# CFSAN-Biostatistics/snp-pipeline

Measured on AMD Instinct MI355X. Metric: consensus_bases_called_per_sec, higher is better.
Workload: dtype u8; 1 GPU; BASELINE configs[3] shard (125 samples/GPU x 5000000 bp x 30x synthetic pileups, 49878 SNP sites, 1500 SNP records per sample; the reference bundles no pileups); step = site-record gather + site union, one batched scan launch + one call launch, 4-bit pack, row all-gather, all-pairs distance tiles, row-band exchange; samples_total=125, samples_this_rank=125, genome_bp=5000000, snp_sites=49878, pileup_bytes_this_rank=54061520755, parallelism=samples sharded over 1 rank(s)

## Files before the change

snp_pipeline_amd/csrc/prims.h:

```cpp
#pragma once

#include <hip/hip_runtime.h>
#include <stdint.h>

__device__ __forceinline__ uint32_t wave_inclusive_sum(uint32_t v) {
    v += (uint32_t)__builtin_amdgcn_update_dpp(0, (int)v, 0x111, 0xF, 0xF, false);
    v += (uint32_t)__builtin_amdgcn_update_dpp(0, (int)v, 0x112, 0xF, 0xF, false);
    v += (uint32_t)__builtin_amdgcn_update_dpp(0, (int)v, 0x114, 0xF, 0xF, false);
    v += (uint32_t)__builtin_amdgcn_update_dpp(0, (int)v, 0x118, 0xF, 0xF, false);
    v += (uint32_t)__builtin_amdgcn_update_dpp(0, (int)v, 0x142, 0xA, 0xF, false);
    v += (uint32_t)__builtin_amdgcn_update_dpp(0, (int)v, 0x143, 0xC, 0xF, false);
    return v;
}

__device__ __forceinline__ uint32_t block_exclusive_sum(uint32_t v, uint32_t *lds, uint32_t &total) {
    const uint32_t lane = threadIdx.x & 63, wave = threadIdx.x >> 6, n_waves = (blockDim.x + 63) >> 6;
    const uint32_t incl = wave_inclusive_sum(v);
    if (lane == 63) lds[wave] = incl;
    __syncthreads();
    if (wave == 0) {
        const uint32_t w = lane < n_waves ? lds[lane] : 0u;
        const uint32_t wi = wave_inclusive_sum(w);
        if (lane < n_waves) lds[lane] = wi - w;
        if (lane == 63) lds[16] = wi;
    }
    __syncthreads();
    total = lds[16];
    return lds[wave] + incl - v;
}

#define PRIM_SCAN_THREADS 1024
#define PRIM_SCAN_ITEMS 8
#define PRIM_SCAN_BLOCK (PRIM_SCAN_THREADS * PRIM_SCAN_ITEMS)

static inline uint32_t prim_scan_blocks(uint64_t n) { return (uint32_t)((n + PRIM_SCAN_BLOCK - 1) / PRIM_SCAN_BLOCK); }
static inline size_t prim_scan_workspace_words(uint64_t n) { return (size_t)prim_scan_blocks(n) + 2; }

__global__ __launch_bounds__(PRIM_SCAN_THREADS) static void k_prim_scan_reduce(const uint32_t *in, uint64_t n, uint32_t *block_sums) {
    __shared__ uint32_t lds[17];
    const uint64_t base = (uint64_t)blockIdx.x * PRIM_SCAN_BLOCK + (uint64_t)threadIdx.x * PRIM_SCAN_ITEMS;
    uint32_t s = 0;
#pragma unroll
    for (int k = 0; k < PRIM_SCAN_ITEMS; ++k) s += base + k < n ? in[base + k] : 0u;
    uint32_t total;
    (void)block_exclusive_sum(s, lds, total);
    if (threadIdx.x == 0) block_sums[blockIdx.x] = total;
}

__global__ __launch_bounds__(PRIM_SCAN_THREADS) static void k_prim_scan_spine(uint32_t *block_sums, uint32_t n_blocks, uint32_t *total) {
    __shared__ uint32_t lds[17];
    uint32_t carry = 0;
    for (uint32_t b0 = 0; b0 < n_blocks; b0 += PRIM_SCAN_THREADS) {
        const uint32_t i = b0 + threadIdx.x;
        const uint32_t v = i < n_blocks ? block_sums[i] : 0u;
        uint32_t t;
        const uint32_t ex = block_exclusive_sum(v, lds, t);
        if (i < n_blocks) block_sums[i] = carry + ex;
        carry += t;
        __syncthreads();
    }
    if (threadIdx.x == 0) total[0] = carry;
}

__global__ __launch_bounds__(PRIM_SCAN_THREADS) static void k_prim_scan_apply(const uint32_t *in, uint32_t *out, uint64_t n, const uint32_t *block_sums) {
    __shared__ uint32_t lds[17];
    const uint64_t base = (uint64_t)blockIdx.x * PRIM_SCAN_BLOCK + (uint64_t)threadIdx.x * PRIM_SCAN_ITEMS;
    uint32_t v[PRIM_SCAN_ITEMS], s = 0;
#pragma unroll
    for (int k = 0; k < PRIM_SCAN_ITEMS; ++k) { v[k] = base + k < n ? in[base + k] : 0u; s += v[k]; }
    uint32_t total;
    uint32_t run = block_sums[blockIdx.x] + block_exclusive_sum(s, lds, total);
#pragma unroll
    for (int k = 0; k < PRIM_SCAN_ITEMS; ++k) {
        if (base + k < n) out[base + k] = run;
        run += v[k];
    }
}

static inline void prim_exclusive_scan_u32(hipStream_t st, const uint32_t *in, uint32_t *out, uint64_t n, uint32_t *ws, uint32_t **d_total) {
    const uint32_t nb = prim_scan_blocks(n);
    uint32_t *total = ws + nb;
    if (d_total) *d_total = total;
    if (n == 0) { (void)hipMemsetAsync(total, 0, 4, st); return; }
    k_prim_scan_reduce<<<nb, PRIM_SCAN_THREADS, 0, st>>>(in, n, ws);
    k_prim_scan_spine<<<1, PRIM_SCAN_THREADS, 0, st>>>(ws, nb, total);
    k_prim_scan_apply<<<nb, PRIM_SCAN_THREADS, 0, st>>>(in, out, n, ws);
}

#define PRIM_GSCAN_THREADS 256
#define PRIM_GSCAN_ITEMS 8
#define PRIM_GSCAN_BLOCK (PRIM_GSCAN_THREADS * PRIM_GSCAN_ITEMS)
static inline uint32_t prim_gscan_blocks(uint64_t n) { return (uint32_t)((n + PRIM_GSCAN_BLOCK - 1) / PRIM_GSCAN_BLOCK); }

template <typename T, typename Op>
__device__ __forceinline__ T block_inclusive_scan_generic(T v, T *lds, Op op) {
    lds[threadIdx.x] = v;
    __syncthreads();
    for (uint32_t d = 1; d < PRIM_GSCAN_THREADS; d <<= 1) {
        T other = v;
        const bool take = threadIdx.x >= d;
        if (take) other = lds[threadIdx.x - d];
        __syncthreads();
        if (take) { v = op(other, v); lds[threadIdx.x] = v; }
        __syncthreads();
    }
    return v;
}

template <typename T, typename Op, int kPhase>
__global__ __launch_bounds__(PRIM_GSCAN_THREADS) static void k_prim_gscan(const T *in, T *out, uint64_t n, T *aggr, uint32_t n_blocks, Op op) {
    __shared__ T lds[PRIM_GSCAN_THREADS];
    if (kPhase == 1) {
        T carry = T();
        bool have = false;
        for (uint32_t b0 = 0; b0 < n_blocks; b0 += PRIM_GSCAN_THREADS) {
            const uint32_t i = b0 + threadIdx.x;
            const uint32_t last = n_blocks - b0 < PRIM_GSCAN_THREADS ? n_blocks - b0 - 1 : PRIM_GSCAN_THREADS - 1;
            T v = aggr[i < n_blocks ? i : n_blocks - 1];
            if (i >= n_blocks) v = aggr[n_blocks - 1];
            T s = block_inclusive_scan_generic(v, lds, op);
            if (have) s = op(carry, s);
            if (i < n_blocks) aggr[i] = s;
            __syncthreads();
            lds[threadIdx.x] = s;
            __syncthreads();
            carry = lds[last];
            have = true;
            __syncthreads();
        }
        return;
    }
    const uint64_t base = (uint64_t)blockIdx.x * PRIM_GSCAN_BLOCK + (uint64_t)threadIdx.x * PRIM_GSCAN_ITEMS;
    T v[PRIM_GSCAN_ITEMS];
    const uint64_t left = base < n ? n - base : 0;
    const int cnt = left >= PRIM_GSCAN_ITEMS ? PRIM_GSCAN_ITEMS : (int)left;
#pragma unroll
    for (int k = 0; k < PRIM_GSCAN_ITEMS; ++k) if (k < cnt) v[k] = in[base + k];
#pragma unroll
    for (int k = 1; k < PRIM_GSCAN_ITEMS; ++k) if (k < cnt) v[k] = op(v[k - 1], v[k]);
    __shared__ uint8_t ok[PRIM_GSCAN_THREADS];
    ok[threadIdx.x] = cnt > 0;
    T a = cnt > 0 ? v[cnt - 1] : T();
    lds[threadIdx.x] = a;
    __syncthreads();
    bool a_ok = cnt > 0;
    for (uint32_t d = 1; d < PRIM_GSCAN_THREADS; d <<= 1) {
        T other = a;
        bool o_ok = false;
        const bool take = threadIdx.x >= d;
        if (take) { other = lds[threadIdx.x - d]; o_ok = ok[threadIdx.x - d]; }
        __syncthreads();
        if (take && o_ok) { a = a_ok ? op(other, a) : other; a_ok = true; lds[threadIdx.x] = a; ok[threadIdx.x] = 1; }
        __syncthreads();
    }
    if (kPhase == 0) {
        if (threadIdx.x == PRIM_GSCAN_THREADS - 1) aggr[blockIdx.x] = a;
        return;
    }
    T pre = T();
    bool pre_ok = false;
    if (threadIdx.x > 0) { pre = lds[threadIdx.x - 1]; pre_ok = ok[threadIdx.x - 1]; }
    if (blockIdx.x > 0) { const T bp = aggr[blockIdx.x - 1]; pre = pre_ok ? op(bp, pre) : bp; pre_ok = true; }
#pragma unroll
    for (int k = 0; k < PRIM_GSCAN_ITEMS; ++k) if (k < cnt) out[base + k] = pre_ok ? op(pre, v[k]) : v[k];
}

template <typename T, typename Op>
static inline void prim_inclusive_scan(hipStream_t st, const T *in, T *out, uint64_t n, T *aggr, Op op) {
    if (n == 0) return;
    const uint32_t nb = prim_gscan_blocks(n);
    k_prim_gscan<T, Op, 0><<<nb, PRIM_GSCAN_THREADS, 0, st>>>(in, out, n, aggr, nb, op);
    k_prim_gscan<T, Op, 1><<<1, PRIM_GSCAN_THREADS, 0, st>>>(in, out, n, aggr, nb, op);
    k_prim_gscan<T, Op, 2><<<nb, PRIM_GSCAN_THREADS, 0, st>>>(in, out, n, aggr, nb, op);
}

#define PRIM_SORT_TILE 2048
#ifndef PRIM_SORT_THREADS
#define PRIM_SORT_THREADS 1024
#endif

template <typename T, typename Less>
__global__ __launch_bounds__(PRIM_SORT_THREADS) static void k_prim_sort_check(const T *in, uint64_t n, uint32_t *unsorted, Less less) {
    bool bad = false;
    for (uint64_t i = (uint64_t)blockIdx.x * blockDim.x + threadIdx.x; i + 1 < n; i += (uint64_t)gridDim.x * blockDim.x)
        bad = bad || less(in[i + 1], in[i]);
    if (__ballot(bad) && (threadIdx.x & 63) == 0) *unsorted = 1u;
}

template <typename T, typename Less>
__global__ __launch_bounds__(PRIM_SORT_THREADS) static void k_prim_sort_tiles(const T *in, T *out, T *out_if_sorted, uint64_t n,
                                                                             const uint32_t *unsorted, Less less) {
    __shared__ T tile[PRIM_SORT_TILE];
    __shared__ uint16_t idx[PRIM_SORT_TILE];
    const uint64_t base = (uint64_t)blockIdx.x * PRIM_SORT_TILE;
    const uint32_t cnt = n - base < PRIM_SORT_TILE ? (uint32_t)(n - base) : PRIM_SORT_TILE;
    if (*unsorted == 0) {
        for (uint32_t i = threadIdx.x; i < cnt; i += PRIM_SORT_THREADS) out_if_sorted[base + i] = in[base + i];
        return;
    }
    for (uint32_t i = threadIdx.x; i < PRIM_SORT_TILE; i += PRIM_SORT_THREADS) {
        if (i < cnt) tile[i] = in[base + i];
        idx[i] = i < cnt ? (uint16_t)i : (uint16_t)0xFFFFu;
    }
    __syncthreads();
    auto before = [&](uint16_t a, uint16_t b) -> bool {
        if (a == 0xFFFFu || b == 0xFFFFu) return a != 0xFFFFu && b == 0xFFFFu;
        if (less(tile[a], tile[b])) return true;
        if (less(tile[b], tile[a])) return false;
        return a < b;
    };
    for (uint32_t k = 2; k <= PRIM_SORT_TILE; k <<= 1)
        for (uint32_t j = k >> 1; j > 0; j >>= 1) {
            for (uint32_t t = threadIdx.x; t < PRIM_SORT_TILE / 2; t += PRIM_SORT_THREADS) {
                const uint32_t lo = ((t & ~(j - 1)) << 1) | (t & (j - 1)), hi = lo | j;
                const bool up = (lo & k) == 0;
                const uint16_t a = idx[lo], b = idx[hi];
                if (before(b, a) == up) { idx[lo] = b; idx[hi] = a; }
            }
            __syncthreads();
        }
    for (uint32_t i = threadIdx.x; i < cnt; i += PRIM_SORT_THREADS) out[base + i] = tile[idx[i]];
}

template <typename T, typename Less>
__global__ __launch_bounds__(PRIM_SORT_THREADS) static void k_prim_merge_pass(const T *in, T *out, uint64_t n, uint64_t run,
                                                                             const uint32_t *unsorted, Less less) {
    __shared__ T stage[PRIM_SORT_TILE];
    __shared__ uint64_t split[2];
    if (*unsorted == 0) return;
    const uint64_t o0 = (uint64_t)blockIdx.x * PRIM_SORT_TILE;
    const uint64_t pair0 = o0 / (2 * run) * (2 * run);
    const uint64_t a_begin = pair0, a_len = n - pair0 < run ? n - pair0 : run;
    const uint64_t b_begin = pair0 + a_len, b_len = n - b_begin < run ? n - b_begin : run;
    const uint64_t d0 = o0 - pair0, total = a_len + b_len;
    const uint64_t d1 = d0 + PRIM_SORT_TILE < total ? d0 + PRIM_SORT_TILE : total;
    const T *A = in + a_begin, *B = in + b_begin;
    if (threadIdx.x < 2) {
        const uint64_t d = threadIdx.x ? d1 : d0;
        uint64_t lo = d > b_len ? d - b_len : 0, hi = d < a_len ? d : a_len;
        while (lo < hi) {
            const uint64_t mid = (lo + hi) >> 1;
            if (!less(B[d - 1 - mid], A[mid])) lo = mid + 1; else hi = mid;
        }
        split[threadIdx.x] = lo;
    }
    __syncthreads();
    const uint64_t a0 = split[0], a1 = split[1], b0 = d0 - a0, b1 = d1 - a1;
    const uint32_t na = (uint32_t)(a1 - a0), nb = (uint32_t)(b1 - b0);
    for (uint32_t i = threadIdx.x; i < na + nb; i += PRIM_SORT_THREADS) stage[i] = i < na ? A[a0 + i] : B[b0 + (i - na)];
    __syncthreads();
    for (uint32_t i = threadIdx.x; i < na + nb; i += PRIM_SORT_THREADS) {
        const T v = stage[i];
        uint32_t lo, hi;
        if (i < na) {
            lo = 0; hi = nb;
            while (lo < hi) { const uint32_t mid = (lo + hi) >> 1; if (less(stage[na + mid], v)) lo = mid + 1; else hi = mid; }
            out[o0 + i + lo] = v;
        } else {
            lo = 0; hi = na;
            while (lo < hi) { const uint32_t mid = (lo + hi) >> 1; if (!less(v, stage[mid])) lo = mid + 1; else hi = mid; }
            out[o0 + (i - na) + lo] = v;
        }
    }
}

static inline uint32_t prim_sort_passes(uint64_t n) {
    uint32_t p = 0;
    for (uint64_t run = PRIM_SORT_TILE; run < n; run <<= 1) ++p;
    return p;
}
template <typename T, typename Less>
static inline T *prim_sort(hipStream_t st, const T *in, T *buf_a, T *buf_b, uint64_t n, uint32_t *flag, Less less) {
    const uint32_t passes = prim_sort_passes(n);
    T *final_buf = (passes & 1) ? buf_b : buf_a;
    if (n == 0) return final_buf;
    const uint32_t tiles = (uint32_t)((n + PRIM_SORT_TILE - 1) / PRIM_SORT_TILE);
    (void)hipMemsetAsync(flag, 0, 4, st);
    const uint64_t cb = (n + PRIM_SORT_THREADS - 1) / PRIM_SORT_THREADS;
    k_prim_sort_check<T, Less><<<(unsigned)(cb < 2048 ? cb : 2048), PRIM_SORT_THREADS, 0, st>>>(in, n, flag, less);
    k_prim_sort_tiles<T, Less><<<tiles, PRIM_SORT_THREADS, 0, st>>>(in, buf_a, final_buf, n, flag, less);
    T *src = buf_a, *dst = buf_b;
    for (uint64_t run = PRIM_SORT_TILE; run < n; run <<= 1) {
        k_prim_merge_pass<T, Less><<<tiles, PRIM_SORT_THREADS, 0, st>>>(src, dst, n, run, flag, less);
        T *t = src; src = dst; dst = t;
    }
    return final_buf;
}
```

snp_pipeline_amd/csrc/regions.hip:

```cpp
#include <string.h>

#include <vector>

#include "internal.h"
#include "prims.h"

namespace {

inline size_t up256(size_t x) { return (x + 255) / 256 * 256; }
inline unsigned nblk(uint64_t n) { return (unsigned)((n + 255) / 256); }

#define R_TRY(ctx, expr)                                                                                \
    do {                                                                                                \
        hipError_t e_ = (expr);                                                                         \
        if (e_ != hipSuccess)                                                                           \
            return snpgpu_set_error((ctx), SNPGPU_E_HIP, "%s failed: %s", #expr, hipGetErrorString(e_)); \
    } while (0)

#define REG_ERR_POSITION 1u
#define REG_ERR_INTERVAL 2u

struct U64Less { __device__ bool operator()(const uint64_t &a, const uint64_t &b) const { return a < b; } };

#define MAX_RULES 64
struct Rules { int32_t max_snps[MAX_RULES], window[MAX_RULES]; uint32_t n; };

__device__ __forceinline__ uint32_t seg_of(const uint32_t *seg_off, uint32_t n_segs, uint32_t i) {
    uint32_t lo = 0, hi = n_segs;
    while (hi - lo > 1) { uint32_t mid = (lo + hi) >> 1; if (seg_off[mid] <= i) lo = mid; else hi = mid; }
    return lo;
}

__global__ void k_seg_keys(const int64_t *pos, const uint32_t *seg_off, uint32_t n_segs, uint32_t n_pos, uint64_t *keys, uint32_t *out_n) {
    uint32_t i = blockIdx.x * blockDim.x + threadIdx.x;
    if (i >= n_pos) return;
    int64_t p = pos[i];
    if (p < 0 || p >= (1ll << 40)) { atomicOr(&out_n[1], REG_ERR_POSITION); p = 0; }
    keys[i] = ((uint64_t)seg_of(seg_off, n_segs, i) << 40) | (uint64_t)p;
}

__global__ void k_dense_flags(const uint64_t *keys, const uint32_t *seg_off, uint32_t n_segs, uint32_t n_pos, Rules rules, uint32_t *flag) {
    uint64_t g = (uint64_t)blockIdx.x * blockDim.x + threadIdx.x;
    if (g >= (uint64_t)n_pos * rules.n) return;
    const uint32_t i = (uint32_t)(g / rules.n), r = (uint32_t)(g % rules.n);
    const uint32_t end = seg_off[seg_of(seg_off, n_segs, i) + 1];
    const int64_t m = rules.max_snps[r], mask = (1ll << 40) - 1;
    uint32_t f = 0;
    if (m >= 0 && (uint64_t)i + (uint64_t)m < end) f = ((int64_t)(keys[i] & mask) + (int64_t)rules.window[r] - 1 >= (int64_t)(keys[i + m] & mask)) ? 1u : 0u;
    flag[g] = f;
}

__global__ void k_dense_emit(const uint64_t *keys, uint32_t n_pos, Rules rules, const uint32_t *flag, const uint32_t *slot,
                             int64_t *out_start, int64_t *out_end, uint32_t *out_seg) {
    uint64_t g = (uint64_t)blockIdx.x * blockDim.x + threadIdx.x;
    if (g >= (uint64_t)n_pos * rules.n || !flag[g]) return;
    const uint32_t i = (uint32_t)(g / rules.n), r = (uint32_t)(g % rules.n);
    const uint64_t mask = (1ull << 40) - 1;
    const uint32_t o = slot[g];
    out_start[o] = (int64_t)(keys[i] & mask);
    out_end[o] = (int64_t)(keys[i + rules.max_snps[r]] & mask);
    out_seg[o] = (uint32_t)(keys[i] >> 40);
}

__global__ void k_copy_word(const uint32_t *src, uint32_t *dst) { *dst = *src; }

size_t dense_ws_bytes(uint32_t n_pos, uint32_t n_rules) {
    const uint64_t total = (uint64_t)n_pos * n_rules;
    return 3 * up256(8ull * n_pos) + 256 + 2 * up256(4 * total) + up256(4 * prim_scan_workspace_words(total)) + 256;
}

int dense_enqueue(snpgpu_ctx *ctx, const int64_t *d_pos, const uint32_t *d_seg_off, uint32_t n_segs, uint32_t n_pos, const Rules &rules,
                  int64_t *d_out_start, int64_t *d_out_end, uint32_t *d_out_seg, uint32_t *d_out_n, char *ws) {
    hipStream_t st = ctx->stream;
    const uint64_t total = (uint64_t)n_pos * rules.n;
    size_t o = 0;
    uint64_t *keys = (uint64_t *)(ws + o); o += up256(8ull * n_pos);
    uint64_t *ka = (uint64_t *)(ws + o); o += up256(8ull * n_pos);
    uint64_t *kb = (uint64_t *)(ws + o); o += up256(8ull * n_pos);
    uint32_t *sflag = (uint32_t *)(ws + o); o += 256;
    uint32_t *flag = (uint32_t *)(ws + o); o += up256(4 * total);
    uint32_t *slot = (uint32_t *)(ws + o); o += up256(4 * total);
    uint32_t *scan_ws = (uint32_t *)(ws + o);
    R_TRY(ctx, hipMemsetAsync(d_out_n, 0, 8, st));
    if (n_pos && rules.n) {
        k_seg_keys<<<nblk(n_pos), 256, 0, st>>>(d_pos, d_seg_off, n_segs, n_pos, keys, d_out_n);
        const uint64_t *sorted = prim_sort<uint64_t, U64Less>(st, keys, ka, kb, n_pos, sflag, U64Less());
        k_dense_flags<<<nblk(total), 256, 0, st>>>(sorted, d_seg_off, n_segs, n_pos, rules, flag);
        uint32_t *d_total = nullptr;
        prim_exclusive_scan_u32(st, flag, slot, total, scan_ws, &d_total);
        k_dense_emit<<<nblk(total), 256, 0, st>>>(sorted, n_pos, rules, flag, slot, d_out_start, d_out_end, d_out_seg);
        k_copy_word<<<1, 1, 0, st>>>(d_total, d_out_n);
    }
    R_TRY(ctx, hipGetLastError());
    return SNPGPU_OK;
}

int make_rules(snpgpu_ctx *ctx, const int32_t *max_snps, const int32_t *window, uint32_t n_rules, Rules &rules) {
    if (n_rules > MAX_RULES) return snpgpu_set_error(ctx, SNPGPU_E_UNSUPPORTED, "more than %d dense-window rules", MAX_RULES);
    if (n_rules && (!max_snps || !window)) return snpgpu_set_error(ctx, SNPGPU_E_ARG, "null dense-window argument");
    memset(&rules, 0, sizeof rules);
    rules.n = n_rules;
    for (uint32_t r = 0; r < n_rules; ++r) { rules.max_snps[r] = max_snps[r]; rules.window[r] = window[r]; }
    return SNPGPU_OK;
}

struct Ival { uint32_t group, pad; int64_t start, end; };
struct IvalLess {
    __device__ bool operator()(const Ival &a, const Ival &b) const {
        if (a.group != b.group) return a.group < b.group;
        if (a.start != b.start) return a.start < b.start;
        return a.end < b.end;
    }
};
struct GroupMax { int64_t maxend; uint32_t group, pad; };
struct GroupMaxOp {
    __device__ GroupMax operator()(const GroupMax &a, const GroupMax &b) const {
        GroupMax r;
        r.group = b.group; r.pad = 0;
        r.maxend = (a.group == b.group && a.maxend > b.maxend) ? a.maxend : b.maxend;
        return r;
    }
};

__global__ void k_ival_pack(const uint32_t *group, const int64_t *start, const int64_t *end, uint32_t n, Ival *out, uint32_t *out_n) {
    uint32_t i = blockIdx.x * blockDim.x + threadIdx.x;
    if (i >= n) return;
    Ival v;
    v.group = group[i]; v.pad = 0; v.start = start[i]; v.end = end[i];
    if (v.start > v.end) atomicOr(&out_n[1], REG_ERR_INTERVAL);
    out[i] = v;
}

__global__ void k_ival_ends(const Ival *sorted, uint32_t n, GroupMax *gm) {
    uint32_t i = blockIdx.x * blockDim.x + threadIdx.x;
    if (i < n) { GroupMax g; g.group = sorted[i].group; g.pad = 0; g.maxend = sorted[i].end; gm[i] = g; }
}

__global__ void k_ival_heads(const Ival *sorted, const GroupMax *run, uint32_t n, uint32_t *head) {
    uint32_t i = blockIdx.x * blockDim.x + threadIdx.x;
    if (i >= n) return;
    uint32_t h = 1;
    if (i > 0 && run[i - 1].group == sorted[i].group) {
        const int64_t le = run[i - 1].maxend;
        h = (le == INT64_MAX || sorted[i].start <= le + 1) ? 0u : 1u;
    }
    head[i] = h;
}

__global__ void k_ival_emit(const Ival *sorted, const GroupMax *run, const uint32_t *head, const uint32_t *slot, uint32_t n,
                            uint32_t *out_group, int64_t *out_start, int64_t *out_end) {
    uint32_t i = blockIdx.x * blockDim.x + threadIdx.x;
    if (i >= n) return;
    const uint32_t o = slot[i] + head[i] - 1;
    if (head[i]) { out_group[o] = sorted[i].group; out_start[o] = sorted[i].start; }
    if (i + 1 == n || head[i + 1]) out_end[o] = run[i].maxend;
}

size_t merge_regions_ws_bytes(uint32_t n) {
    return 3 * up256(sizeof(Ival) * (size_t)n) + 256 + 2 * up256(sizeof(GroupMax) * (size_t)n) + up256(sizeof(GroupMax) * (size_t)prim_gscan_blocks(n)) +
           2 * up256(4ull * n) + up256(4 * prim_scan_workspace_words(n)) + 256;
}

int merge_regions_enqueue(snpgpu_ctx *ctx, const uint32_t *d_group, const int64_t *d_start, const int64_t *d_end, uint32_t n,
                          uint32_t *d_out_group, int64_t *d_out_start, int64_t *d_out_end, uint32_t *d_out_n, char *ws) {
    hipStream_t st = ctx->stream;
    size_t o = 0;
    Ival *iv = (Ival *)(ws + o); o += up256(sizeof(Ival) * (size_t)n);
    Ival *ia = (Ival *)(ws + o); o += up256(sizeof(Ival) * (size_t)n);
    Ival *ib = (Ival *)(ws + o); o += up256(sizeof(Ival) * (size_t)n);
    uint32_t *sflag = (uint32_t *)(ws + o); o += 256;
    GroupMax *gm = (GroupMax *)(ws + o); o += up256(sizeof(GroupMax) * (size_t)n);
    GroupMax *run = (GroupMax *)(ws + o); o += up256(sizeof(GroupMax) * (size_t)n);
    GroupMax *aggr = (GroupMax *)(ws + o); o += up256(sizeof(GroupMax) * (size_t)prim_gscan_blocks(n));
    uint32_t *head = (uint32_t *)(ws + o); o += up256(4ull * n);
    uint32_t *slot = (uint32_t *)(ws + o); o += up256(4ull * n);
    uint32_t *scan_ws = (uint32_t *)(ws + o);
    R_TRY(ctx, hipMemsetAsync(d_out_n, 0, 8, st));
    if (n) {
        k_ival_pack<<<nblk(n), 256, 0, st>>>(d_group, d_start, d_end, n, iv, d_out_n);
        const Ival *sorted = prim_sort<Ival, IvalLess>(st, iv, ia, ib, n, sflag, IvalLess());
        k_ival_ends<<<nblk(n), 256, 0, st>>>(sorted, n, gm);
        prim_inclusive_scan<GroupMax, GroupMaxOp>(st, gm, run, n, aggr, GroupMaxOp());
        k_ival_heads<<<nblk(n), 256, 0, st>>>(sorted, run, n, head);
        uint32_t *d_total = nullptr;
        prim_exclusive_scan_u32(st, head, slot, n, scan_ws, &d_total);
        k_ival_emit<<<nblk(n), 256, 0, st>>>(sorted, run, head, slot, n, d_out_group, d_out_start, d_out_end);
        k_copy_word<<<1, 1, 0, st>>>(d_total, d_out_n);
    }
    R_TRY(ctx, hipGetLastError());
    return SNPGPU_OK;
}

__global__ void k_in_regions(const uint32_t *pos_group, const int64_t *pos, uint32_t n, const uint32_t *reg_off,
                             const int64_t *rs, const int64_t *re, uint32_t n_groups, uint8_t *out) {
    uint32_t i = blockIdx.x * blockDim.x + threadIdx.x;
    if (i >= n) return;
    uint32_t g = pos_group[i];
    uint8_t f = 0;
    if (g < n_groups) {
        int64_t p = pos[i];
        uint32_t lo = reg_off[g], hi = reg_off[g + 1];
        while (lo < hi) {
            uint32_t mid = (lo + hi) >> 1;
            if (rs[mid] <= p) lo = mid + 1; else hi = mid;
        }
        if (lo > reg_off[g]) f = re[lo - 1] >= p;
    }
    out[i] = f;
}

struct Pair { uint64_t key; uint32_t samp, pad; };
struct PairLess {
    __device__ bool operator()(const Pair &a, const Pair &b) const { return a.key != b.key ? a.key < b.key : a.samp < b.samp; }
};

__global__ void k_pair_pack(const uint64_t *keys, const uint32_t *samp, uint32_t n, Pair *out) {
    uint32_t i = blockIdx.x * blockDim.x + threadIdx.x;
    if (i < n) { Pair p; p.key = keys[i]; p.samp = samp[i]; p.pad = 0; out[i] = p; }
}

__global__ void k_sites_flags(const Pair *sorted, uint32_t n, uint32_t *new_key, uint32_t *new_pair) {
    uint32_t i = blockIdx.x * blockDim.x + threadIdx.x;
    if (i >= n) return;
    const bool nk = i == 0 || sorted[i].key != sorted[i - 1].key;
    new_key[i] = nk;
    new_pair[i] = nk || sorted[i].samp != sorted[i - 1].samp;
}

__global__ void k_sites_emit(const Pair *sorted, uint32_t n, const uint32_t *new_key, const uint32_t *new_pair, const uint32_t *key_slot,
                             const uint32_t *pair_slot, const uint32_t *n_keys, const uint32_t *n_pairs, uint64_t *out_unique,
                             uint32_t *out_off, uint32_t *out_carrier, uint32_t *out_n) {
    uint32_t i = blockIdx.x * blockDim.x + threadIdx.x;
    if (i == 0) { out_n[0] = *n_keys; out_n[1] = *n_pairs; out_off[*n_keys] = *n_pairs; }
    if (i >= n) return;
    if (new_pair[i]) out_carrier[pair_slot[i]] = sorted[i].samp;
    if (new_key[i]) { out_unique[key_slot[i]] = sorted[i].key; out_off[key_slot[i]] = pair_slot[i]; }
}

size_t merge_sites_ws_bytes(uint64_t n) {
    return 3 * up256(sizeof(Pair) * (size_t)n) + 256 + 4 * up256(4ull * n) + 2 * up256(4 * prim_scan_workspace_words(n)) + 256;
}

int merge_sites_enqueue(snpgpu_ctx *ctx, const uint64_t *d_keys, const uint32_t *d_samp, uint32_t n, uint64_t *d_out_unique,
                        uint32_t *d_out_off, uint32_t *d_out_carrier, uint32_t *d_out_n, char *ws) {
    hipStream_t st = ctx->stream;
    size_t o = 0;
    Pair *pr = (Pair *)(ws + o); o += up256(sizeof(Pair) * (size_t)n);
    Pair *pa = (Pair *)(ws + o); o += up256(sizeof(Pair) * (size_t)n);
    Pair *pb = (Pair *)(ws + o); o += up256(sizeof(Pair) * (size_t)n);
    uint32_t *sflag = (uint32_t *)(ws + o); o += 256;
    uint32_t *nk = (uint32_t *)(ws + o); o += up256(4ull * n);
    uint32_t *np = (uint32_t *)(ws + o); o += up256(4ull * n);
    uint32_t *ks = (uint32_t *)(ws + o); o += up256(4ull * n);
    uint32_t *ps = (uint32_t *)(ws + o); o += up256(4ull * n);
    uint32_t *scan1 = (uint32_t *)(ws + o); o += up256(4 * prim_scan_workspace_words(n));
    uint32_t *scan2 = (uint32_t *)(ws + o);
    R_TRY(ctx, hipMemsetAsync(d_out_n, 0, 8, st));
    R_TRY(ctx, hipMemsetAsync(d_out_off, 0, 4, st));
    if (n) {
        k_pair_pack<<<nblk(n), 256, 0, st>>>(d_keys, d_samp, n, pr);
        const Pair *sorted = prim_sort<Pair, PairLess>(st, pr, pa, pb, n, sflag, PairLess());
        k_sites_flags<<<nblk(n), 256, 0, st>>>(sorted, n, nk, np);
        uint32_t *t_keys = nullptr, *t_pairs = nullptr;
        prim_exclusive_scan_u32(st, nk, ks, n, scan1, &t_keys);
        prim_exclusive_scan_u32(st, np, ps, n, scan2, &t_pairs);
        k_sites_emit<<<nblk(n), 256, 0, st>>>(sorted, n, nk, np, ks, ps, t_keys, t_pairs, d_out_unique, d_out_off, d_out_carrier, d_out_n);
    }
    R_TRY(ctx, hipGetLastError());
    return SNPGPU_OK;
}

int region_error(snpgpu_ctx *ctx, uint32_t bits) {
    if (bits & REG_ERR_POSITION) return snpgpu_set_error(ctx, SNPGPU_E_UNSUPPORTED, "SNP position outside [0, 2^40)");
    if (bits & REG_ERR_INTERVAL) return snpgpu_set_error(ctx, SNPGPU_E_UNSUPPORTED, "interval with start > end");
    return SNPGPU_OK;
}

}

extern "C" {

int snpgpu_dense_windows_dev(snpgpu_ctx *ctx, const int64_t *d_positions, const uint32_t *d_seg_off, uint32_t n_segs, uint32_t n_pos,
                             const int32_t *max_snps, const int32_t *window, uint32_t n_rules, int64_t *d_out_start,
                             int64_t *d_out_end, uint32_t *d_out_seg, uint32_t *d_out_n) {
    if (!ctx || !d_out_n) return SNPGPU_E_ARG;
    Rules rules;
    int rc = make_rules(ctx, max_snps, window, n_rules, rules);
    if (rc) return rc;
    if ((uint64_t)n_pos * n_rules > 0x7FFFFFFFull) return snpgpu_set_error(ctx, SNPGPU_E_UNSUPPORTED, "too many (position, rule) pairs");
    if (n_segs >= (1u << 24)) return snpgpu_set_error(ctx, SNPGPU_E_UNSUPPORTED, "too many segments");
    if (n_pos && (!d_positions || !d_seg_off || !d_out_start || !d_out_end || !d_out_seg)) return snpgpu_set_error(ctx, SNPGPU_E_ARG, "null dense-window argument");
    R_TRY(ctx, snpgpu_enter(ctx));
    void *ws = nullptr;
    rc = snpgpu_scratch(ctx, dense_ws_bytes(n_pos, n_rules), &ws);
    if (rc) return rc;
    return dense_enqueue(ctx, d_positions, d_seg_off, n_segs, n_pos, rules, d_out_start, d_out_end, d_out_seg, d_out_n, (char *)ws);
}

int snpgpu_merge_regions_dev(snpgpu_ctx *ctx, const uint32_t *d_group, const int64_t *d_start, const int64_t *d_end, uint32_t n,
                             uint32_t *d_out_group, int64_t *d_out_start, int64_t *d_out_end, uint32_t *d_out_n) {
    if (!ctx || !d_out_n) return SNPGPU_E_ARG;
    if (n && (!d_group || !d_start || !d_end || !d_out_group || !d_out_start || !d_out_end)) return snpgpu_set_error(ctx, SNPGPU_E_ARG, "null merge argument");
    R_TRY(ctx, snpgpu_enter(ctx));
    void *ws = nullptr;
    int rc = snpgpu_scratch(ctx, merge_regions_ws_bytes(n), &ws);
    if (rc) return rc;
    return merge_regions_enqueue(ctx, d_group, d_start, d_end, n, d_out_group, d_out_start, d_out_end, d_out_n, (char *)ws);
}

int snpgpu_in_regions_dev(snpgpu_ctx *ctx, const uint32_t *d_pos_group, const int64_t *d_positions, uint32_t n_pos,
                          const uint32_t *d_reg_off, const int64_t *d_reg_start, const int64_t *d_reg_end, uint32_t n_groups,
                          uint8_t *d_out_flag) {
    if (!ctx) return SNPGPU_E_ARG;
    if (n_pos == 0) return SNPGPU_OK;
    if (!d_pos_group || !d_positions || !d_out_flag || (n_groups && !d_reg_off)) return snpgpu_set_error(ctx, SNPGPU_E_ARG, "null in_regions argument");
    R_TRY(ctx, snpgpu_enter(ctx));
    k_in_regions<<<nblk(n_pos), 256, 0, ctx->stream>>>(d_pos_group, d_positions, n_pos, d_reg_off, d_reg_start, d_reg_end, n_groups, d_out_flag);
    R_TRY(ctx, hipGetLastError());
    return SNPGPU_OK;
}

int snpgpu_merge_sites_dev(snpgpu_ctx *ctx, const uint64_t *d_keys, const uint32_t *d_sample_of_key, uint32_t n,
                           uint64_t *d_out_unique, uint32_t *d_out_off, uint32_t *d_out_carrier, uint32_t *d_out_n) {
    if (!ctx || !d_out_n || !d_out_off) return SNPGPU_E_ARG;
    if (n > 0x7FFFFFFFu) return snpgpu_set_error(ctx, SNPGPU_E_UNSUPPORTED, "too many site records");
    if (n && (!d_keys || !d_sample_of_key || !d_out_unique || !d_out_carrier)) return snpgpu_set_error(ctx, SNPGPU_E_ARG, "null merge_sites argument");
    R_TRY(ctx, snpgpu_enter(ctx));
    void *ws = nullptr;
    int rc = snpgpu_scratch(ctx, merge_sites_ws_bytes(n), &ws);
    if (rc) return rc;
    return merge_sites_enqueue(ctx, d_keys, d_sample_of_key, n, d_out_unique, d_out_off, d_out_carrier, d_out_n, (char *)ws);
}

int snpgpu_dense_windows(snpgpu_ctx *ctx, const int64_t *positions, const uint32_t *seg_off, uint32_t n_segs,
                         const int32_t *max_snps, const int32_t *window, uint32_t n_rules,
                         int64_t *out_start, int64_t *out_end, uint32_t *out_seg, uint32_t *out_n) {
    if (!ctx || !out_n) return SNPGPU_E_ARG;
    *out_n = 0;
    if (n_segs == 0 || n_rules == 0) return SNPGPU_OK;
    if (!seg_off) return snpgpu_set_error(ctx, SNPGPU_E_ARG, "null dense-window argument");
    const uint32_t n_pos = seg_off[n_segs];
    if (n_pos == 0) return SNPGPU_OK;
    if (!positions || !out_start || !out_end || !out_seg) return snpgpu_set_error(ctx, SNPGPU_E_ARG, "null dense-window argument");
    Rules rules;
    int rc = make_rules(ctx, max_snps, window, n_rules, rules);
    if (rc) return rc;
    const uint64_t total = (uint64_t)n_pos * n_rules;
    if (total > 0x7FFFFFFFull) return snpgpu_set_error(ctx, SNPGPU_E_UNSUPPORTED, "too many (position, rule) pairs");
    if (n_segs >= (1u << 24)) return snpgpu_set_error(ctx, SNPGPU_E_UNSUPPORTED, "too many segments");
    R_TRY(ctx, snpgpu_enter(ctx));
    hipStream_t st = ctx->stream;
    size_t o = 0;
    const size_t o_pos = o; o += up256(8ull * n_pos);
    const size_t o_seg = o; o += up256(4ull * (n_segs + 1));
    const size_t o_os = o; o += up256(8 * total);
    const size_t o_oe = o; o += up256(8 * total);
    const size_t o_og = o; o += up256(4 * total);
    const size_t o_n = o; o += 256;
    const size_t o_ws = o; o += dense_ws_bytes(n_pos, n_rules);
    void *scr = nullptr;
    rc = snpgpu_scratch(ctx, o, &scr);
    if (rc) return rc;
    char *b = (char *)scr;
    R_TRY(ctx, hipMemcpyAsync(b + o_pos, positions, 8ull * n_pos, hipMemcpyHostToDevice, st));
    R_TRY(ctx, hipMemcpyAsync(b + o_seg, seg_off, 4ull * (n_segs + 1), hipMemcpyHostToDevice, st));
    rc = dense_enqueue(ctx, (const int64_t *)(b + o_pos), (const uint32_t *)(b + o_seg), n_segs, n_pos, rules, (int64_t *)(b + o_os),
                       (int64_t *)(b + o_oe), (uint32_t *)(b + o_og), (uint32_t *)(b + o_n), b + o_ws);
    if (rc) return rc;
    uint32_t res[2] = {0, 0};
    R_TRY(ctx, hipMemcpyAsync(res, b + o_n, 8, hipMemcpyDeviceToHost, st));
    R_TRY(ctx, hipStreamSynchronize(st));
    if (res[1]) return region_error(ctx, res[1]);
    if (res[0]) {
        R_TRY(ctx, hipMemcpyAsync(out_start, b + o_os, 8ull * res[0], hipMemcpyDeviceToHost, st));
        R_TRY(ctx, hipMemcpyAsync(out_end, b + o_oe, 8ull * res[0], hipMemcpyDeviceToHost, st));
        R_TRY(ctx, hipMemcpyAsync(out_seg, b + o_og, 4ull * res[0], hipMemcpyDeviceToHost, st));
        R_TRY(ctx, hipStreamSynchronize(st));
    }
    *out_n = res[0];
    return SNPGPU_OK;
}

int snpgpu_merge_regions(snpgpu_ctx *ctx, const uint32_t *group, const int64_t *start, const int64_t *end,
                         uint32_t n, uint32_t *out_group, int64_t *out_start, int64_t *out_end, uint32_t *out_n) {
    if (!ctx || !out_n) return SNPGPU_E_ARG;
    *out_n = 0;
    if (n == 0) return SNPGPU_OK;
    if (!group || !start || !end || !out_group || !out_start || !out_end) return snpgpu_set_error(ctx, SNPGPU_E_ARG, "null merge argument");
    R_TRY(ctx, snpgpu_enter(ctx));
    hipStream_t st = ctx->stream;
    size_t o = 0;
    const size_t o_g = o; o += up256(4ull * n);
    const size_t o_s = o; o += up256(8ull * n);
    const size_t o_e = o; o += up256(8ull * n);
    const size_t o_og = o; o += up256(4ull * n);
    const size_t o_os = o; o += up256(8ull * n);
    const size_t o_oe = o; o += up256(8ull * n);
    const size_t o_n = o; o += 256;
    const size_t o_ws = o; o += merge_regions_ws_bytes(n);
    void *scr = nullptr;
    int rc = snpgpu_scratch(ctx, o, &scr);
    if (rc) return rc;
    char *b = (char *)scr;
    R_TRY(ctx, hipMemcpyAsync(b + o_g, group, 4ull * n, hipMemcpyHostToDevice, st));
    R_TRY(ctx, hipMemcpyAsync(b + o_s, start, 8ull * n, hipMemcpyHostToDevice, st));
    R_TRY(ctx, hipMemcpyAsync(b + o_e, end, 8ull * n, hipMemcpyHostToDevice, st));
    rc = merge_regions_enqueue(ctx, (const uint32_t *)(b + o_g), (const int64_t *)(b + o_s), (const int64_t *)(b + o_e), n,
                               (uint32_t *)(b + o_og), (int64_t *)(b + o_os), (int64_t *)(b + o_oe), (uint32_t *)(b + o_n), b + o_ws);
    if (rc) return rc;
    uint32_t res[2] = {0, 0};
    R_TRY(ctx, hipMemcpyAsync(res, b + o_n, 8, hipMemcpyDeviceToHost, st));
    R_TRY(ctx, hipStreamSynchronize(st));
    if (res[1]) return region_error(ctx, res[1]);
    R_TRY(ctx, hipMemcpyAsync(out_group, b + o_og, 4ull * res[0], hipMemcpyDeviceToHost, st));
    R_TRY(ctx, hipMemcpyAsync(out_start, b + o_os, 8ull * res[0], hipMemcpyDeviceToHost, st));
    R_TRY(ctx, hipMemcpyAsync(out_end, b + o_oe, 8ull * res[0], hipMemcpyDeviceToHost, st));
    R_TRY(ctx, hipStreamSynchronize(st));
    *out_n = res[0];
    return SNPGPU_OK;
}

int snpgpu_in_regions(snpgpu_ctx *ctx, const uint32_t *pos_group, const int64_t *positions, uint32_t n_pos,
                      const uint32_t *reg_off, const int64_t *reg_start, const int64_t *reg_end,
                      uint32_t n_groups, uint8_t *out_flag) {
    if (!ctx) return SNPGPU_E_ARG;
    if (n_pos == 0) return SNPGPU_OK;
    if (!pos_group || !positions || !out_flag || (n_groups && !reg_off)) return snpgpu_set_error(ctx, SNPGPU_E_ARG, "null in_regions argument");
    R_TRY(ctx, snpgpu_enter(ctx));
    hipStream_t st = ctx->stream;
    const uint32_t n_reg = n_groups ? reg_off[n_groups] : 0;
    size_t o = 0;
    const size_t o_g = o; o += up256(4ull * n_pos);
    const size_t o_p = o; o += up256(8ull * n_pos);
    const size_t o_off = o; o += up256(4ull * (n_groups + 1));
    const size_t o_rs = o; o += up256(8ull * n_reg);
    const size_t o_re = o; o += up256(8ull * n_reg);
    const size_t o_out = o; o += up256(n_pos);
    void *scr = nullptr;
    int rc = snpgpu_scratch(ctx, o + 256, &scr);
    if (rc) return rc;
    char *b = (char *)scr;
    R_TRY(ctx, hipMemcpyAsync(b + o_g, pos_group, 4ull * n_pos, hipMemcpyHostToDevice, st));
    R_TRY(ctx, hipMemcpyAsync(b + o_p, positions, 8ull * n_pos, hipMemcpyHostToDevice, st));
    if (n_groups) R_TRY(ctx, hipMemcpyAsync(b + o_off, reg_off, 4ull * (n_groups + 1), hipMemcpyHostToDevice, st));
    if (n_reg) {
        R_TRY(ctx, hipMemcpyAsync(b + o_rs, reg_start, 8ull * n_reg, hipMemcpyHostToDevice, st));
        R_TRY(ctx, hipMemcpyAsync(b + o_re, reg_end, 8ull * n_reg, hipMemcpyHostToDevice, st));
    }
    k_in_regions<<<nblk(n_pos), 256, 0, st>>>((const uint32_t *)(b + o_g), (const int64_t *)(b + o_p), n_pos, (const uint32_t *)(b + o_off),
                                              (const int64_t *)(b + o_rs), (const int64_t *)(b + o_re), n_groups, (uint8_t *)(b + o_out));
    R_TRY(ctx, hipMemcpyAsync(out_flag, b + o_out, n_pos, hipMemcpyDeviceToHost, st));
    R_TRY(ctx, hipStreamSynchronize(st));
    return SNPGPU_OK;
}

int snpgpu_merge_sites(snpgpu_ctx *ctx, const uint64_t *keys, const uint32_t *sample_of_key, size_t n,
                       uint64_t *out_unique, uint32_t *out_off, uint32_t *out_carrier,
                       uint32_t *out_n_unique, uint32_t *out_n_carrier) {
    if (!ctx || !out_n_unique || !out_n_carrier) return SNPGPU_E_ARG;
    *out_n_unique = *out_n_carrier = 0;
    if (out_off) out_off[0] = 0;
    if (n == 0) return SNPGPU_OK;
    if (n > 0x7FFFFFFFull) return snpgpu_set_error(ctx, SNPGPU_E_UNSUPPORTED, "too many site records");
    if (!keys || !sample_of_key || !out_unique || !out_off || !out_carrier) return snpgpu_set_error(ctx, SNPGPU_E_ARG, "null merge_sites argument");
    R_TRY(ctx, snpgpu_enter(ctx));
    hipStream_t st = ctx->stream;
    const uint32_t m = (uint32_t)n;
    size_t o = 0;
    const size_t o_k = o; o += up256(8ull * m);
    const size_t o_s = o; o += up256(4ull * m);
    const size_t o_u = o; o += up256(8ull * m);
    const size_t o_off = o; o += up256(4ull * (m + 1));
    const size_t o_c = o; o += up256(4ull * m);
    const size_t o_n = o; o += 256;
    const size_t o_ws = o; o += merge_sites_ws_bytes(m);
    void *scr = nullptr;
    int rc = snpgpu_scratch(ctx, o, &scr);
    if (rc) return rc;
    char *b = (char *)scr;
    R_TRY(ctx, hipMemcpyAsync(b + o_k, keys, 8ull * m, hipMemcpyHostToDevice, st));
    R_TRY(ctx, hipMemcpyAsync(b + o_s, sample_of_key, 4ull * m, hipMemcpyHostToDevice, st));
    rc = merge_sites_enqueue(ctx, (const uint64_t *)(b + o_k), (const uint32_t *)(b + o_s), m, (uint64_t *)(b + o_u), (uint32_t *)(b + o_off),
                             (uint32_t *)(b + o_c), (uint32_t *)(b + o_n), b + o_ws);
    if (rc) return rc;
    uint32_t res[2] = {0, 0};
    R_TRY(ctx, hipMemcpyAsync(res, b + o_n, 8, hipMemcpyDeviceToHost, st));
    R_TRY(ctx, hipStreamSynchronize(st));
    R_TRY(ctx, hipMemcpyAsync(out_unique, b + o_u, 8ull * res[0], hipMemcpyDeviceToHost, st));
    R_TRY(ctx, hipMemcpyAsync(out_off, b + o_off, 4ull * (res[0] + 1), hipMemcpyDeviceToHost, st));
    R_TRY(ctx, hipMemcpyAsync(out_carrier, b + o_c, 4ull * res[1], hipMemcpyDeviceToHost, st));
    R_TRY(ctx, hipStreamSynchronize(st));
    *out_n_unique = res[0];
    *out_n_carrier = res[1];
    return SNPGPU_OK;
}

}

size_t snpgpu_merge_sites_ws_bytes(uint64_t n) { return merge_sites_ws_bytes(n); }

int snpgpu_enqueue_merge_sites_ws(snpgpu_ctx *ctx, const uint64_t *d_keys, const uint32_t *d_sample_of_key, uint32_t n, uint64_t *d_out_unique, uint32_t *d_out_off,
                                  uint32_t *d_out_carrier, uint32_t *d_out_n, void *d_ws) {
    if (n > 0x7FFFFFFFu) return snpgpu_set_error(ctx, SNPGPU_E_UNSUPPORTED, "too many site records");
    return merge_sites_enqueue(ctx, d_keys, d_sample_of_key, n, d_out_unique, d_out_off, d_out_carrier, d_out_n, (char *)d_ws);
}
```

Before: 704.9 million bases/s.

## Fuse pair packing into sort, replace flag scans with block-count emit, parallel merge splits

Site-union merging now feeds keys and sample IDs straight into the sort through a load functor, which removes the separate pack kernel and its buffer. The separate flag, two-scan and emit sequence becomes a block-count kernel plus an emit kernel that recomputes flags and takes block offsets, either self-computed or via a spine scan. This cuts launches and full-length intermediate arrays. The merge pass also finds its split points with a 64-way parallel probe search instead of a serial binary search in one thread, adding syncs per round.

```diff
diff --git a/snp_pipeline_amd/csrc/prims.h b/snp_pipeline_amd/csrc/prims.h
--- a/snp_pipeline_amd/csrc/prims.h
+++ b/snp_pipeline_amd/csrc/prims.h
@@ -178,28 +178,37 @@
 #ifndef PRIM_SORT_THREADS
 #define PRIM_SORT_THREADS 1024
 #endif
-
-template <typename T, typename Less>
-__global__ __launch_bounds__(PRIM_SORT_THREADS) static void k_prim_sort_check(const T *in, uint64_t n, uint32_t *unsorted, Less less) {
+#define PRIM_SPLIT_PROBES 64
+#define PRIM_SPLIT_WAVES (PRIM_SPLIT_PROBES / 64)
+static_assert(PRIM_SPLIT_PROBES % 64 == 0 && 2 * PRIM_SPLIT_PROBES <= PRIM_SORT_THREADS, "a wave probes for one diagonal only");
+
+template <typename T>
+struct PrimLoadArray {
+    const T *in;
+    __device__ __forceinline__ T operator()(uint64_t i) const { return in[i]; }
+};
+
+template <typename T, typename Less, typename Load>
+__global__ __launch_bounds__(PRIM_SORT_THREADS) static void k_prim_sort_check(Load load, uint64_t n, uint32_t *unsorted, Less less) {
     bool bad = false;
     for (uint64_t i = (uint64_t)blockIdx.x * blockDim.x + threadIdx.x; i + 1 < n; i += (uint64_t)gridDim.x * blockDim.x)
-        bad = bad || less(in[i + 1], in[i]);
+        bad = bad || less(load(i + 1), load(i));
     if (__ballot(bad) && (threadIdx.x & 63) == 0) *unsorted = 1u;
 }
 
-template <typename T, typename Less>
-__global__ __launch_bounds__(PRIM_SORT_THREADS) static void k_prim_sort_tiles(const T *in, T *out, T *out_if_sorted, uint64_t n,
+template <typename T, typename Less, typename Load>
+__global__ __launch_bounds__(PRIM_SORT_THREADS) static void k_prim_sort_tiles(Load load, T *out, T *out_if_sorted, uint64_t n,
                                                                              const uint32_t *unsorted, Less less) {
     __shared__ T tile[PRIM_SORT_TILE];
     __shared__ uint16_t idx[PRIM_SORT_TILE];
     const uint64_t base = (uint64_t)blockIdx.x * PRIM_SORT_TILE;
     const uint32_t cnt = n - base < PRIM_SORT_TILE ? (uint32_t)(n - base) : PRIM_SORT_TILE;
     if (*unsorted == 0) {
-        for (uint32_t i = threadIdx.x; i < cnt; i += PRIM_SORT_THREADS) out_if_sorted[base + i] = in[base + i];
+        for (uint32_t i = threadIdx.x; i < cnt; i += PRIM_SORT_THREADS) out_if_sorted[base + i] = load(base + i);
         return;
     }
     for (uint32_t i = threadIdx.x; i < PRIM_SORT_TILE; i += PRIM_SORT_THREADS) {
-        if (i < cnt) tile[i] = in[base + i];
+        if (i < cnt) tile[i] = load(base + i);
         idx[i] = i < cnt ? (uint16_t)i : (uint16_t)0xFFFFu;
     }
     __syncthreads();
@@ -226,7 +235,7 @@
 __global__ __launch_bounds__(PRIM_SORT_THREADS) static void k_prim_merge_pass(const T *in, T *out, uint64_t n, uint64_t run,
                                                                              const uint32_t *unsorted, Less less) {
     __shared__ T stage[PRIM_SORT_TILE];
-    __shared__ uint64_t split[2];
+    __shared__ uint32_t fails[2][2 * PRIM_SPLIT_WAVES];
     if (*unsorted == 0) return;
     const uint64_t o0 = (uint64_t)blockIdx.x * PRIM_SORT_TILE;
     const uint64_t pair0 = o0 / (2 * run) * (2 * run);
@@ -235,17 +244,29 @@
     const uint64_t d0 = o0 - pair0, total = a_len + b_len;
     const uint64_t d1 = d0 + PRIM_SORT_TILE < total ? d0 + PRIM_SORT_TILE : total;
     const T *A = in + a_begin, *B = in + b_begin;
-    if (threadIdx.x < 2) {
-        const uint64_t d = threadIdx.x ? d1 : d0;
-        uint64_t lo = d > b_len ? d - b_len : 0, hi = d < a_len ? d : a_len;
-        while (lo < hi) {
-            const uint64_t mid = (lo + hi) >> 1;
-            if (!less(B[d - 1 - mid], A[mid])) lo = mid + 1; else hi = mid;
+    const uint32_t half = threadIdx.x / PRIM_SPLIT_PROBES, probe = threadIdx.x % PRIM_SPLIT_PROBES;
+    uint64_t rlo[2], rhi[2];
+    rlo[0] = d0 > b_len ? d0 - b_len : 0; rhi[0] = d0 < a_len ? d0 : a_len;
+    rlo[1] = d1 > b_len ? d1 - b_len : 0; rhi[1] = d1 < a_len ? d1 : a_len;
+    for (uint32_t round = 0; rlo[0] < rhi[0] || rlo[1] < rhi[1]; ++round) {
+        const uint64_t d = half ? d1 : d0, l = half ? rlo[1] : rlo[0], h = half ? rhi[1] : rhi[0];
+        const uint64_t step = (h - l + PRIM_SPLIT_PROBES - 1) / PRIM_SPLIT_PROBES;
+        const uint64_t a = l + (uint64_t)(probe + 1) * step - 1;
+        const bool fail = half < 2 && step && a < h && !less(B[d - 1 - a], A[a]);
+        const uint64_t m = __ballot(fail);
+        if ((threadIdx.x & 63) == 0 && half < 2) fails[round & 1][threadIdx.x >> 6] = (uint32_t)__popcll(m);
+        __syncthreads();
+#pragma unroll
+        for (int s = 0; s < 2; ++s) {
+            uint32_t c = 0;
+#pragma unroll
+            for (int w = 0; w < PRIM_SPLIT_WAVES; ++w) c += fails[round & 1][s * PRIM_SPLIT_WAVES + w];
+            const uint64_t st = (rhi[s] - rlo[s] + PRIM_SPLIT_PROBES - 1) / PRIM_SPLIT_PROBES;
+            const uint64_t first_ok = rlo[s] + (uint64_t)(c + 1) * st - 1;
+            if (st) { rlo[s] += (uint64_t)c * st; if (first_ok < rhi[s]) rhi[s] = first_ok; }
         }
-        split[threadIdx.x] = lo;
-    }
-    __syncthreads();
-    const uint64_t a0 = split[0], a1 = split[1], b0 = d0 - a0, b1 = d1 - a1;
+    }
+    const uint64_t a0 = rlo[0], a1 = rlo[1], b0 = d0 - a0, b1 = d1 - a1;
     const uint32_t na = (uint32_t)(a1 - a0), nb = (uint32_t)(b1 - b0);
     for (uint32_t i = threadIdx.x; i < na + nb; i += PRIM_SORT_THREADS) stage[i] = i < na ? A[a0 + i] : B[b0 + (i - na)];
     __syncthreads();
@@ -269,16 +290,16 @@
     for (uint64_t run = PRIM_SORT_TILE; run < n; run <<= 1) ++p;
     return p;
 }
-template <typename T, typename Less>
-static inline T *prim_sort(hipStream_t st, const T *in, T *buf_a, T *buf_b, uint64_t n, uint32_t *flag, Less less) {
+template <typename T, typename Less, typename Load>
+static inline T *prim_sort_from(hipStream_t st, Load load, T *buf_a, T *buf_b, uint64_t n, uint32_t *flag, Less less) {
     const uint32_t passes = prim_sort_passes(n);
     T *final_buf = (passes & 1) ? buf_b : buf_a;
     if (n == 0) return final_buf;
     const uint32_t tiles = (uint32_t)((n + PRIM_SORT_TILE - 1) / PRIM_SORT_TILE);
     (void)hipMemsetAsync(flag, 0, 4, st);
     const uint64_t cb = (n + PRIM_SORT_THREADS - 1) / PRIM_SORT_THREADS;
-    k_prim_sort_check<T, Less><<<(unsigned)(cb < 2048 ? cb : 2048), PRIM_SORT_THREADS, 0, st>>>(in, n, flag, less);
-    k_prim_sort_tiles<T, Less><<<tiles, PRIM_SORT_THREADS, 0, st>>>(in, buf_a, final_buf, n, flag, less);
+    k_prim_sort_check<T, Less, Load><<<(unsigned)(cb < 2048 ? cb : 2048), PRIM_SORT_THREADS, 0, st>>>(load, n, flag, less);
+    k_prim_sort_tiles<T, Less, Load><<<tiles, PRIM_SORT_THREADS, 0, st>>>(load, buf_a, final_buf, n, flag, less);
     T *src = buf_a, *dst = buf_b;
     for (uint64_t run = PRIM_SORT_TILE; run < n; run <<= 1) {
         k_prim_merge_pass<T, Less><<<tiles, PRIM_SORT_THREADS, 0, st>>>(src, dst, n, run, flag, less);
@@ -286,3 +307,7 @@
     }
     return final_buf;
 }
+template <typename T, typename Less>
+static inline T *prim_sort(hipStream_t st, const T *in, T *buf_a, T *buf_b, uint64_t n, uint32_t *flag, Less less) {
+    return prim_sort_from<T, Less, PrimLoadArray<T>>(st, PrimLoadArray<T>{in}, buf_a, buf_b, n, flag, less);
+}
diff --git a/snp_pipeline_amd/csrc/regions.hip b/snp_pipeline_amd/csrc/regions.hip
--- a/snp_pipeline_amd/csrc/regions.hip
+++ b/snp_pipeline_amd/csrc/regions.hip
@@ -214,27 +214,94 @@
     __device__ bool operator()(const Pair &a, const Pair &b) const { return a.key != b.key ? a.key < b.key : a.samp < b.samp; }
 };
 
-__global__ void k_pair_pack(const uint64_t *keys, const uint32_t *samp, uint32_t n, Pair *out) {
-    uint32_t i = blockIdx.x * blockDim.x + threadIdx.x;
-    if (i < n) { Pair p; p.key = keys[i]; p.samp = samp[i]; p.pad = 0; out[i] = p; }
-}
-
-__global__ void k_sites_flags(const Pair *sorted, uint32_t n, uint32_t *new_key, uint32_t *new_pair) {
-    uint32_t i = blockIdx.x * blockDim.x + threadIdx.x;
-    if (i >= n) return;
-    const bool nk = i == 0 || sorted[i].key != sorted[i - 1].key;
-    new_key[i] = nk;
-    new_pair[i] = nk || sorted[i].samp != sorted[i - 1].samp;
-}
-
-__global__ void k_sites_emit(const Pair *sorted, uint32_t n, const uint32_t *new_key, const uint32_t *new_pair, const uint32_t *key_slot,
-                             const uint32_t *pair_slot, const uint32_t *n_keys, const uint32_t *n_pairs, uint64_t *out_unique,
-                             uint32_t *out_off, uint32_t *out_carrier, uint32_t *out_n) {
-    uint32_t i = blockIdx.x * blockDim.x + threadIdx.x;
-    if (i == 0) { out_n[0] = *n_keys; out_n[1] = *n_pairs; out_off[*n_keys] = *n_pairs; }
-    if (i >= n) return;
-    if (new_pair[i]) out_carrier[pair_slot[i]] = sorted[i].samp;
-    if (new_key[i]) { out_unique[key_slot[i]] = sorted[i].key; out_off[key_slot[i]] = pair_slot[i]; }
+struct PairLoad {
+    const uint64_t *keys; const uint32_t *samp;
+    __device__ __forceinline__ Pair operator()(uint64_t i) const { Pair p; p.key = keys[i]; p.samp = samp[i]; p.pad = 0; return p; }
+};
+
+#define SITES_THREADS 256
+#define SITES_ITEMS 4
+#define SITES_BLOCK (SITES_THREADS * SITES_ITEMS)
+#define SITES_SELF_MAX ((uint32_t)SITES_THREADS * SITES_BLOCK)
+#define SITES_SPINE_THREADS 1024
+static_assert(SITES_BLOCK < (1 << 16), "a block's two flag counts share one word");
+
+inline uint32_t sites_blocks(uint64_t n) { return (uint32_t)((n + SITES_BLOCK - 1) / SITES_BLOCK); }
+
+__device__ __forceinline__ uint32_t sites_flags(const Pair *sorted, uint32_t n, uint32_t first, Pair *v, uint32_t *f) {
+    uint32_t sum = 0;
+    Pair prev = {0, 0, 0};
+    if (first > 0 && first < n) prev = sorted[first - 1];
+#pragma unroll
+    for (int k = 0; k < SITES_ITEMS; ++k) {
+        const uint32_t i = first + k;
+        f[k] = 0;
+        if (i < n) {
+            v[k] = sorted[i];
+            const bool nk = i == 0 || v[k].key != prev.key;
+            f[k] = nk ? 0x10001u : (v[k].samp != prev.samp ? 1u : 0u);
+            prev = v[k];
+        }
+        sum += f[k];
+    }
+    return sum;
+}
+
+__global__ __launch_bounds__(SITES_THREADS) void k_sites_count(const Pair *sorted, uint32_t n, uint32_t *tot_keys, uint32_t *tot_pairs) {
+    __shared__ uint32_t lds[17];
+    Pair v[SITES_ITEMS];
+    uint32_t f[SITES_ITEMS], total;
+    const uint32_t s = sites_flags(sorted, n, blockIdx.x * SITES_BLOCK + threadIdx.x * SITES_ITEMS, v, f);
+    (void)block_exclusive_sum(s, lds, total);
+    if (threadIdx.x == 0) { tot_keys[blockIdx.x] = total >> 16; tot_pairs[blockIdx.x] = total & 0xFFFFu; }
+}
+
+__global__ __launch_bounds__(SITES_SPINE_THREADS) void k_sites_spine(uint32_t *tot_keys, uint32_t *tot_pairs, uint32_t n_blocks) {
+    __shared__ uint32_t lds[17];
+    uint32_t carry_k = 0, carry_p = 0;
+    for (uint32_t b0 = 0; b0 < n_blocks; b0 += SITES_SPINE_THREADS) {
+        const uint32_t i = b0 + threadIdx.x;
+        const uint32_t vk = i < n_blocks ? tot_keys[i] : 0u, vp = i < n_blocks ? tot_pairs[i] : 0u;
+        uint32_t tk, tp;
+        const uint32_t ek = block_exclusive_sum(vk, lds, tk);
+        __syncthreads();
+        const uint32_t ep = block_exclusive_sum(vp, lds, tp);
+        if (i < n_blocks) { tot_keys[i] = carry_k + ek; tot_pairs[i] = carry_p + ep; }
+        carry_k += tk; carry_p += tp;
+        __syncthreads();
+    }
+}
+
+template <bool kSelf>
+__global__ __launch_bounds__(SITES_THREADS) void k_sites_emit(const Pair *sorted, uint32_t n, const uint32_t *tot_keys, const uint32_t *tot_pairs,
+                                                              uint64_t *out_unique, uint32_t *out_off, uint32_t *out_carrier, uint32_t *out_n) {
+    __shared__ uint32_t lds[17];
+    uint32_t key0, pair0;
+    if (kSelf) {
+        const bool mine = threadIdx.x < blockIdx.x;
+        (void)block_exclusive_sum(mine ? tot_keys[threadIdx.x] : 0u, lds, key0);
+        __syncthreads();
+        (void)block_exclusive_sum(mine ? tot_pairs[threadIdx.x] : 0u, lds, pair0);
+        __syncthreads();
+    } else {
+        key0 = tot_keys[blockIdx.x]; pair0 = tot_pairs[blockIdx.x];
+    }
+    Pair v[SITES_ITEMS];
+    uint32_t f[SITES_ITEMS], total;
+    const uint32_t first = blockIdx.x * SITES_BLOCK + threadIdx.x * SITES_ITEMS;
+    const uint32_t s = sites_flags(sorted, n, first, v, f);
+    const uint32_t ex = block_exclusive_sum(s, lds, total);
+    uint32_t ks = key0 + (ex >> 16), ps = pair0 + (ex & 0xFFFFu);
+#pragma unroll
+    for (int k = 0; k < SITES_ITEMS; ++k) {
+        if (f[k] & 1u) out_carrier[ps] = v[k].samp;
+        if (f[k] >> 16) { out_unique[ks] = v[k].key; out_off[ks] = ps; }
+        ks += f[k] >> 16; ps += f[k] & 1u;
+    }
+    if (blockIdx.x == gridDim.x - 1 && threadIdx.x == 0) {
+        const uint32_t n_keys = key0 + (total >> 16), n_pairs = pair0 + (total & 0xFFFFu);
+        out_n[0] = n_keys; out_n[1] = n_pairs; out_off[n_keys] = n_pairs;
+    }
 }
 
 size_t merge_sites_ws_bytes(uint64_t n) {
@@ -244,27 +311,26 @@
 int merge_sites_enqueue(snpgpu_ctx *ctx, const uint64_t *d_keys, const uint32_t *d_samp, uint32_t n, uint64_t *d_out_unique,
                         uint32_t *d_out_off, uint32_t *d_out_carrier, uint32_t *d_out_n, char *ws) {
     hipStream_t st = ctx->stream;
-    size_t o = 0;
-    Pair *pr = (Pair *)(ws + o); o += up256(sizeof(Pair) * (size_t)n);
+    const uint32_t nb = sites_blocks(n);
+    size_t o = 0;
     Pair *pa = (Pair *)(ws + o); o += up256(sizeof(Pair) * (size_t)n);
     Pair *pb = (Pair *)(ws + o); o += up256(sizeof(Pair) * (size_t)n);
     uint32_t *sflag = (uint32_t *)(ws + o); o += 256;
-    uint32_t *nk = (uint32_t *)(ws + o); o += up256(4ull * n);
-    uint32_t *np = (uint32_t *)(ws + o); o += up256(4ull * n);
-    uint32_t *ks = (uint32_t *)(ws + o); o += up256(4ull * n);
-    uint32_t *ps = (uint32_t *)(ws + o); o += up256(4ull * n);
-    uint32_t *scan1 = (uint32_t *)(ws + o); o += up256(4 * prim_scan_workspace_words(n));
-    uint32_t *scan2 = (uint32_t *)(ws + o);
-    R_TRY(ctx, hipMemsetAsync(d_out_n, 0, 8, st));
-    R_TRY(ctx, hipMemsetAsync(d_out_off, 0, 4, st));
-    if (n) {
-        k_pair_pack<<<nblk(n), 256, 0, st>>>(d_keys, d_samp, n, pr);
-        const Pair *sorted = prim_sort<Pair, PairLess>(st, pr, pa, pb, n, sflag, PairLess());
-        k_sites_flags<<<nblk(n), 256, 0, st>>>(sorted, n, nk, np);
-        uint32_t *t_keys = nullptr, *t_pairs = nullptr;
-        prim_exclusive_scan_u32(st, nk, ks, n, scan1, &t_keys);
-        prim_exclusive_scan_u32(st, np, ps, n, scan2, &t_pairs);
-        k_sites_emit<<<nblk(n), 256, 0, st>>>(sorted, n, nk, np, ks, ps, t_keys, t_pairs, d_out_unique, d_out_off, d_out_carrier, d_out_n);
+    uint32_t *tk = (uint32_t *)(ws + o); o += up256(4ull * nb);
+    uint32_t *tp = (uint32_t *)(ws + o);
+    if (n == 0) {
+        R_TRY(ctx, hipMemsetAsync(d_out_n, 0, 8, st));
+        R_TRY(ctx, hipMemsetAsync(d_out_off, 0, 4, st));
+        return SNPGPU_OK;
+    }
+    PairLoad load; load.keys = d_keys; load.samp = d_samp;
+    const Pair *sorted = prim_sort_from<Pair, PairLess, PairLoad>(st, load, pa, pb, n, sflag, PairLess());
+    k_sites_count<<<nb, SITES_THREADS, 0, st>>>(sorted, n, tk, tp);
+    if (n <= SITES_SELF_MAX) {
+        k_sites_emit<true><<<nb, SITES_THREADS, 0, st>>>(sorted, n, tk, tp, d_out_unique, d_out_off, d_out_carrier, d_out_n);
+    } else {
+        k_sites_spine<<<1, SITES_SPINE_THREADS, 0, st>>>(tk, tp, nb);
+        k_sites_emit<false><<<nb, SITES_THREADS, 0, st>>>(sorted, n, tk, tp, d_out_unique, d_out_off, d_out_carrier, d_out_n);
     }
     R_TRY(ctx, hipGetLastError());
     return SNPGPU_OK;
```

After: 708.0 million bases/s, median of 6. No clear change (+0.4%).
